# bcgsc/NanoSim

Measured on AMD Instinct MI355X. Metric: simulated reads/sec (genome mode, mean 8 kb), higher is better.
Workload: dtype u8

## Files before the change

### nanosim_amd/csrc/ns_chain.h

```cpp
#pragma once
#include "ns_device.h"

struct Tabs {
    const uint64_t *w;
    NS_DEV const double *d(uint32_t off) const { return reinterpret_cast<const double *>(w + off); }
    NS_DEV const uint64_t *q(uint32_t off) const { return w + off; }
    NS_DEV const uint16_t *h(uint32_t off) const { return reinterpret_cast<const uint16_t *>(w + off); }
    NS_DEV const uint32_t *u(uint32_t off) const { return reinterpret_cast<const uint32_t *>(w + off); }
    NS_DEV const int32_t *i(uint32_t off) const { return reinterpret_cast<const int32_t *>(w + off); }
};

template <class V>
NS_DEV int32_t ecdf_lookup_g(const double *__restrict__ hi, const V *__restrict__ vhi, uint32_t n,
                                                 double vlo0, const uint16_t *__restrict__ guide, uint32_t u) {
    double p = u32_to_p(u);
    uint32_t s = guide[u >> 24];
    if (s < n) {
        const double h0 = hi[s], h1 = hi[min(s + 1, n - 1)];
        if (p > h0) {
            ++s;
            if (s < n && p > h1) { ++s; while (s < n && p > hi[s]) ++s; }
        }
    }
    if (s >= n) { s = n - 1; p = hi[s]; }
    const uint32_t sm = s ? s - 1 : 0;
    const double hs = hi[s], hp = hi[sm], vs = (double)vhi[s], vp = (double)vhi[sm];
    const double plo = s ? hp : 0.0;
    const double vlo = s ? vp : vlo0;
    return (int32_t)floor((p - plo) / (hs - plo) * (vs - vlo) + vlo);
}

NS_DEV void mix_record(const Tabs &T, const ChainTab &c, uint32_t type, uint32_t comp, uint32_t &go, uint32_t &n, uint32_t &h) {
    const uint64_t *r = T.w + c.mix_rec + 2u * (2u * type + comp);
    const uint64_t r0 = r[0], r1 = r[1];
    go = (uint32_t)r0; n = (uint32_t)(r0 >> 32); h = (uint32_t)r1;
}
NS_DEV int32_t run_length_t(const Tabs &T, const ChainTab &c, int type, uint32_t u_mix, uint32_t u_len) {
    const int comp = ((uint64_t)u_mix < T.q(c.mix_w)[type]) ? 0 : 1;
    uint32_t go, n, h;
    mix_record(T, c, (uint32_t)type, (uint32_t)comp, go, n, h);
    const uint64_t u = u_len;
    uint32_t v = reinterpret_cast<const uint8_t *>(T.w)[8u * h + ns_clz32(~u_len)];
    while (v + 1 < n && u >= T.w[go + v]) ++v;
    return (int32_t)v + 1;
}

struct EvSink32 {
    ns_event *ev;
    uint32_t cap, n;
    int32_t shift;
    uint32_t last_ins_len;
    bool overflow;
    bool range;
    uint2 *stg;
    uint32_t stride;
};
#ifndef NS_CHAIN_BLOCK
#define NS_CHAIN_BLOCK 256
#endif
NS_DEV void ev_flush4(EvSink32 &s, uint32_t first) {
    const uint2 e0 = s.stg[0], e1 = s.stg[s.stride], e2 = s.stg[2u * s.stride], e3 = s.stg[3u * s.stride];
    uint4 *dst = reinterpret_cast<uint4 *>(s.ev + first);
    dst[0] = make_uint4(e0.x, e0.y, e1.x, e1.y); dst[1] = make_uint4(e2.x, e2.y, e3.x, e3.y);
}
NS_DEV void ev_flush_tail(EvSink32 &s) {
    if (s.stg && (s.n & 3u) && s.n < s.cap) ev_flush4(s, s.n & ~3u);
}
NS_DEV bool ev_shift_fits(int32_t shift) { return (uint32_t)(shift + NS_EV_SHIFT_BIAS) < 2u * (uint32_t)NS_EV_SHIFT_BIAS; }
NS_DEV void ev_push32(EvSink32 &s, int32_t pos, uint32_t type, int32_t len) {
    uint32_t l = len > (int32_t)NS_EV_LEN_MAX ? NS_EV_LEN_MAX : (uint32_t)len;
    if (len > (int32_t)NS_EV_LEN_MAX || !ev_shift_fits(s.shift)) s.range = true;
    if (s.n < s.cap) {
        ns_event e; e.pos = (uint32_t)pos; e.info = ns_ev_pack(l, type, s.shift);
        if (s.stg) {
            s.stg[(s.n & 3u) * s.stride] = make_uint2(e.pos, e.info);
            if ((s.n & 3u) == 3u) ev_flush4(s, s.n - 3u);
        } else s.ev[s.n] = e;
    } else s.overflow = true;
    if (type == NS_INS) { s.shift += (int32_t)l; s.last_ins_len = l; } else if (type == NS_DEL) s.shift -= (int32_t)l;
    s.n++;
}

struct EList32 { int32_t l_new, middle_ref; };

NS_DEV EList32 chain_error_list_g(const Tabs &T, const ChainTab &c, int32_t m_ref, const ns_key &key, uint32_t seg, uint32_t attempt, EvSink32 &s) {
    int32_t l_new = m_ref, pos = 0, middle_ref = m_ref;
    int state = NS_ST_START;
    u32x4 w = ns_draw(key, ST_EVENT, seg, attempt, 0, 0);
    int32_t prev_match = ecdf_lookup_g(T.d(c.fm_hi), T.d(c.fm_vhi), c.fm_n, c.fm_vlo0, T.h(c.fm_guide), w.x);
    if (prev_match < 2) prev_match = 2;
    pos += prev_match;
    uint32_t it = 1;
    int32_t last_ins_pos = -1;
    const uint64_t *trans = T.q(c.trans);
    const int32_t *bins = T.i(c.mm_bin);
    const uint32_t *seg_off = T.u(c.mm_seg_off);
    const uint8_t *bin_lut = reinterpret_cast<const uint8_t *>(T.w + c.mm_bin_lut);
    u32x4 w_next = ns_draw(key, ST_EVENT, seg, attempt, 1, 0);
    while (pos < middle_ref) {
        w = w_next;
        w_next = ns_draw(key, ST_EVENT, seg, attempt, it + 1, 0);
        const int error = trans_pick_u(trans + 3 * state, w.x);
        int32_t step = run_length_t(T, c, error, w.y, w.z);
        if (error == NS_INS) l_new += step; else if (error == NS_DEL) l_new -= step;
        if (error != NS_INS) {
            ev_push32(s, pos, (uint32_t)error, step);
            pos += step;
            if (pos >= middle_ref) { l_new += pos - middle_ref; middle_ref = pos; }
        } else {
            if (last_ins_pos == pos && s.n > 0) { s.n--; s.shift -= (int32_t)s.last_ins_len; }
            ev_push32(s, pos, NS_INS, step);
            last_ins_pos = pos;
        }
        state = NS_ST_MIS + error;
        uint32_t b;
        if ((uint32_t)prev_match < 256u) b = bin_lut[prev_match];
        else {
            for (b = 0; b < c.mm_nbins; ++b)
                if (bins[2 * b] <= prev_match && prev_match < bins[2 * b + 1]) break;
            if (b >= c.mm_nbins) b = c.mm_nbins - 1;
        }
        const uint32_t o = seg_off[b], ncol = seg_off[b + 1] - o;
        step = ecdf_lookup_g(T.d(c.mm_hi) + o, T.d(c.mm_vhi) + o, ncol, T.d(c.mm_vlo0)[b], T.h(c.mm_guide) + 256 * b, w.w);
        if (prev_match == 0 && step == 0) step = 1;
        prev_match = step;
        if (pos + prev_match > middle_ref) { l_new += pos + prev_match - middle_ref; middle_ref = pos + prev_match; }
        pos += prev_match;
        if (prev_match == 0) state += 3;
        else last_ins_pos = -1;
        ++it;
    }
    return EList32{l_new, middle_ref};
}

struct EvTrack { int32_t max_len, smin, smax; };
NS_DEV EvTrack ev_track_open(const EvSink32 &s) { return EvTrack{0, s.shift, s.shift}; }
NS_DEV void ev_track_close(EvSink32 &s, const EvTrack &t) {
    if (t.max_len > (int32_t)NS_EV_LEN_MAX || !ev_shift_fits(t.smin) || !ev_shift_fits(t.smax)) s.range = true;
    if (s.n > s.cap) s.overflow = true;
}
NS_DEV void ev_push32s(EvSink32 &s, EvTrack &t, int32_t pos, uint32_t type, int32_t len) {
    const uint32_t l = len > (int32_t)NS_EV_LEN_MAX ? NS_EV_LEN_MAX : (uint32_t)len;
    t.max_len = len > t.max_len ? len : t.max_len;
    t.smin = s.shift < t.smin ? s.shift : t.smin; t.smax = s.shift > t.smax ? s.shift : t.smax;
    if (s.n < s.cap) {
        ns_event e; e.pos = (uint32_t)pos; e.info = ns_ev_pack(l, type, s.shift);
        if (s.stg) {
            s.stg[(s.n & 3u) * s.stride] = make_uint2(e.pos, e.info);
            if ((s.n & 3u) == 3u) ev_flush4(s, s.n - 3u);
        } else s.ev[s.n] = e;
    }
    s.shift += type == NS_INS ? (int32_t)l : type == NS_DEL ? -(int32_t)l : 0;
    s.last_ins_len = type == NS_INS ? l : s.last_ins_len;
    s.n++;
}

NS_DEV int32_t run_length_r(const Tabs &T, const ChainTab &c, uint32_t type, uint64_t weight_thr, uint32_t u_mix, uint32_t u_len) {
    const uint32_t comp = (uint64_t)u_mix >= weight_thr ? 1u : 0u;
    const uint64_t *r = T.w + c.mix_rec + 2u * (2u * type + comp);
    const uint64_t r0 = r[0], r1 = r[1];
    const uint32_t go = (uint32_t)r0, rn = (uint32_t)(r0 >> 32);
    const uint64_t uz = u_len;
    uint32_t rv = reinterpret_cast<const uint8_t *>(T.w)[8u * (uint32_t)r1 + ns_clz32(~u_len)];
    const uint64_t ra = T.w[go + rv], rb = T.w[go + rv + 1u];
    const uint32_t c1 = (rv + 1u < rn ? 1u : 0u) & (uz >= ra ? 1u : 0u), c2 = c1 & (rv + 2u < rn ? 1u : 0u) & (uz >= rb ? 1u : 0u);
    rv += c1 + c2;
    if (c2) while (rv + 1u < rn && uz >= T.w[go + rv]) ++rv;
    return (int32_t)rv + 1;
}

#define NS_G_THR(g) ((g) & 0x1ffffffffull)
#define NS_GV_UNIT (1ull << 33)
#define NS_GV_NARROW (1ull << 34)
NS_DEV int32_t ecdf_lookup_gv(const uint64_t *__restrict__ GV, uint32_t n, const uint16_t *__restrict__ guide, uint32_t u,
                              const uint64_t *__restrict__ sub2, const double *__restrict__ hi_g, const double *__restrict__ vhi_g, double vlo0) {
    const uint32_t s0 = guide[u >> 24];
    const uint64_t uu = u;
    const uint32_t sc = min(s0, n - 1u);
    const uint64_t g0 = GV[sc], g1 = GV[sc + 1u];
    const uint32_t k0 = (s0 < n) & (uu >= NS_G_THR(g0)), k1 = k0 & (s0 + 1u < n) & (uu >= NS_G_THR(g1));
    uint64_t g = k0 ? g1 : g0;
    uint32_t s = s0 + k0 + k1;
    if (k1) {
        const uint32_t cell = u >> 24;
        uint32_t hi2 = cell < 255u ? min((uint32_t)guide[cell + 1u], n) : n;
        while (s < hi2) { const uint32_t mid = (s + hi2) >> 1; if (uu >= NS_G_THR(GV[mid])) s = mid + 1u; else hi2 = mid; }
        if (s < n) g = GV[s];
    }
    if (s < n && (g & NS_GV_UNIT)) return (int32_t)(uint32_t)(g >> 35) - 1;
    if (s < n && (g & NS_GV_NARROW)) {
        const uint64_t *t = sub2 + (g >> 35);
        const uint64_t h = t[0];
        const uint32_t nt = (uint32_t)(h >> 32);
        int32_t r = (int32_t)(uint32_t)h - (int32_t)nt;
        for (uint32_t k = 1; k <= nt; ++k) r += uu >= t[k] ? 1 : 0;
        return r;
    }
    double p = u32_to_p(u);
    if (s >= n) { s = n - 1; p = hi_g[s]; }
    const uint32_t sm = s ? s - 1 : 0;
    const double hs = hi_g[s], plo = s ? hi_g[sm] : 0.0, vs = vhi_g[s], vlo = s ? vhi_g[sm] : vlo0;
    return (int32_t)floor((p - plo) / (hs - plo) * (vs - vlo) + vlo);
}

NS_DEV bool ecdf_lookup_pre(const uint64_t *__restrict__ GV, uint32_t n, const uint16_t *__restrict__ guide, uint32_t u,
                            const uint64_t *__restrict__ sub2, int32_t &out) {
    const uint64_t uu = u;
    const uint32_t cell = u >> 24;
    uint32_t s = guide[cell], hi2 = cell < 255u ? min((uint32_t)guide[cell + 1u], n) : n;
    while (s < hi2) { const uint32_t mid = (s + hi2) >> 1; if (uu >= NS_G_THR(GV[mid])) s = mid + 1u; else hi2 = mid; }
    if (s >= n) return false;
    const uint64_t g = GV[s];
    if (g & NS_GV_UNIT) { out = (int32_t)(uint32_t)(g >> 35) - 1; return true; }
    if (g & NS_GV_NARROW) {
        const uint64_t *t = sub2 + (g >> 35);
        const uint64_t h = t[0];
        const uint32_t nt = (uint32_t)(h >> 32);
        int32_t r = (int32_t)(uint32_t)h - (int32_t)nt;
        for (uint32_t k = 1; k <= nt; ++k) r += uu >= t[k] ? 1 : 0;
        out = r;
        return true;
    }
    return false;
}
NS_DEV int32_t next_match_gv(const Tabs &T, const Tabs &TG, const ChainTab &c, int32_t prev_match, uint32_t u) {
    uint32_t b, o, ncol;
    if ((uint32_t)prev_match < 256u) {
        const uint64_t pp = T.q(c.pm_lut)[prev_match];
        int32_t r;
        if (ecdf_lookup_pre(T.q(c.mm_gv) + (uint32_t)pp, (uint32_t)(pp >> 32) & 0xffffffu, T.h(c.mm_guide) + 256u * (uint32_t)(pp >> 56), u, T.q(c.sub2), r)) return r;
        const uint64_t pe = TG.q(c.pm_full)[prev_match];
        b = (uint32_t)(pe >> 56); o = (uint32_t)pe; ncol = (uint32_t)(pe >> 32) & 0xffffffu;
    } else {
        const int32_t *bins = T.i(c.mm_bin);
        const uint32_t *seg_off = T.u(c.mm_seg_off);
        for (b = 0; b < c.mm_nbins; ++b)
            if (bins[2 * b] <= prev_match && prev_match < bins[2 * b + 1]) break;
        if (b >= c.mm_nbins) b = c.mm_nbins - 1;
        const uint64_t pp = T.q(c.pm_bin)[b];
        int32_t r;
        if (ecdf_lookup_pre(T.q(c.mm_gv) + (uint32_t)pp, (uint32_t)(pp >> 32) & 0xffffffu, T.h(c.mm_guide) + 256u * b, u, T.q(c.sub2), r)) return r;
        o = seg_off[b]; ncol = seg_off[b + 1] - o;
    }
    return ecdf_lookup_gv(TG.q(c.mm_gv_full) + o, ncol, T.h(c.mm_guide) + 256u * b, u, TG.q(c.sub2_full), TG.d(c.mm_hi) + o, TG.d(c.mm_vhi) + o, T.d(c.mm_vlo0)[b]);
}

NS_DEV EList32 chain_error_list(const Tabs &T, const Tabs &TG, const ChainTab &c, int32_t m_ref, const ns_key &key,
                                uint32_t seg, uint32_t attempt, EvSink32 &s) {
    int32_t l_new = m_ref, pos = 0, middle_ref = m_ref;
    uint32_t state = NS_ST_START;
    u32x4 w = ns_draw(key, ST_EVENT, seg, attempt, 0, 0);
    int32_t prev_match = ecdf_lookup_gv(TG.q(c.fm_gv), c.fm_n, T.h(c.fm_guide), w.x, TG.q(c.sub2_full), TG.d(c.fm_hi), TG.d(c.fm_vhi), c.fm_vlo0);
    if (prev_match < 2) prev_match = 2;
    pos += prev_match;
    uint32_t it = 1;
    int32_t last_ins_pos = -1;
    const uint64_t *trans = T.q(c.trans);
    const uint64_t *pm = T.q(c.pm_lut);
    const uint64_t *rec = T.q(c.mix_rec);
    const uint64_t *gv = T.q(c.mm_gv);
    const uint16_t *guide = T.h(c.mm_guide);
    const uint8_t *bytes = reinterpret_cast<const uint8_t *>(T.w);
    const uint64_t mw0 = T.q(c.mix_w)[0], mw1 = T.q(c.mix_w)[1], mw2 = T.q(c.mix_w)[2];
    u32x4 w_next = ns_draw(key, ST_EVENT, seg, attempt, 1, 0);
    EvTrack trk = ev_track_open(s);
    while (pos < middle_ref) {
        w = w_next;
        w_next = ns_draw(key, ST_EVENT, seg, attempt, it + 1, 0);
        const uint64_t ux = w.x, uy = w.y, uz = w.z, uw = w.w;
        const uint64_t t0 = trans[3u * state], t1 = trans[3u * state + 1u];
        const uint32_t small = (uint32_t)prev_match < 256u ? 1u : 0u;
        const uint64_t pe = pm[small ? (uint32_t)prev_match : 0u];
        const uint32_t e0 = ux >= t0 ? 1u : 0u, e1 = ux >= t1 ? 1u : 0u;
        const uint32_t error = e0 + (e0 & e1);
        const uint32_t b = (uint32_t)(pe >> 56), o = (uint32_t)pe, ncol = (uint32_t)(pe >> 32) & 0xffffffu;
        const uint64_t mw = error == NS_MIS ? mw0 : error == NS_INS ? mw1 : mw2;
        const uint32_t comp = uy >= mw ? 1u : 0u;
        const uint64_t r0 = rec[2u * (2u * error + comp)], r1 = rec[2u * (2u * error + comp) + 1u];
        const uint32_t s0 = guide[256u * b + (w.w >> 24)];
        const uint32_t go = (uint32_t)r0, rn = (uint32_t)(r0 >> 32);
        uint32_t rv = bytes[8u * (uint32_t)r1 + ns_clz32(~w.z)];
        const uint32_t sc = min(s0, ncol - 1u);
        const uint64_t g0 = gv[o + sc], g1 = gv[o + sc + 1u];
        const uint64_t ra = T.w[go + rv], rb = T.w[go + rv + 1u];
        const uint32_t k0 = (s0 < ncol ? 1u : 0u) & (uw >= NS_G_THR(g0) ? 1u : 0u), k1 = k0 & (s0 + 1u < ncol ? 1u : 0u) & (uw >= NS_G_THR(g1) ? 1u : 0u);
        const uint64_t g = k0 ? g1 : g0;
        const uint32_t fast = small & (s0 + k0 < ncol ? 1u : 0u) & (k1 ^ 1u) & ((g & NS_GV_UNIT) ? 1u : 0u);
        int32_t next = (int32_t)(uint32_t)(g >> 35) - 1;
        const uint32_t c1 = (rv + 1u < rn ? 1u : 0u) & (uz >= ra ? 1u : 0u), c2 = c1 & (rv + 2u < rn ? 1u : 0u) & (uz >= rb ? 1u : 0u);
        rv += c1 + c2;
        if (c2) while (rv + 1u < rn && uz >= T.w[go + rv]) ++rv;
        if (!fast) next = next_match_gv(T, TG, c, prev_match, w.w);
        const int32_t step = (int32_t)rv + 1;
        if (prev_match == 0 && next == 0) next = 1;
        const bool ins = error == NS_INS;
        l_new += ins ? step : error == NS_DEL ? -step : 0;
        const bool coll = ins && last_ins_pos == pos && s.n > 0;
        s.n -= coll ? 1u : 0u; s.shift -= coll ? (int32_t)s.last_ins_len : 0;
        ev_push32s(s, trk, pos, error, step);
        last_ins_pos = ins ? pos : last_ins_pos;
        pos += ins ? 0 : step;
        const bool over = !ins && pos >= middle_ref;
        l_new += over ? pos - middle_ref : 0; middle_ref = over ? pos : middle_ref;
        state = NS_ST_MIS + error;
        prev_match = next;
        if (pos + prev_match > middle_ref) { l_new += pos + prev_match - middle_ref; middle_ref = pos + prev_match; }
        pos += prev_match;
        if (prev_match == 0) state += 3;
        else last_ins_pos = -1;
        ++it;
    }
    ev_track_close(s, trk);
    return EList32{l_new, middle_ref};
}

NS_DEV EList32 chain_unaligned_error_list(const Tabs &T, const ChainTab &c, int32_t m_ref, const ns_key &key,
                                          uint32_t seg, uint32_t attempt, EvSink32 &s) {
    int32_t l_new = m_ref, pos = 0, middle_ref = m_ref;
    int32_t pend_ins = 0;
    if (m_ref <= 0) return EList32{l_new, middle_ref};
    uint32_t it = 0;
    u32x4 w_next = ns_draw(key, ST_UEVENT, seg, attempt, 0, 0);
    const uint64_t mw0 = T.q(c.mix_w)[0], mw1 = T.q(c.mix_w)[1], mw2 = T.q(c.mix_w)[2];
    EvTrack trk = ev_track_open(s);
    while (pos < middle_ref) {
        const u32x4 w = w_next;
        ++it;
        w_next = ns_draw(key, ST_UEVENT, seg, attempt, it, 0);
        const uint64_t ut = w.x;
        const uint32_t type = (ut < ns_thr_lt(0.4)) ? 3u : (ut < ns_thr_lt(0.7)) ? (uint32_t)NS_MIS : (ut < ns_thr_lt(0.85)) ? (uint32_t)NS_INS : (uint32_t)NS_DEL;
        const uint32_t tt = type == 3u ? (uint32_t)NS_MIS : type;
        const int32_t run = run_length_r(T, c, tt, tt == NS_MIS ? mw0 : tt == NS_INS ? mw1 : mw2, w.y, w.z);
        const int32_t step = type == 3u ? 1 : run;
        const bool is_ins = type == NS_INS, is_mis = type == NS_MIS, is_del = type == NS_DEL;
        l_new += is_ins ? step : is_del ? -step : 0;
        const int32_t L = is_ins ? 0 : pend_ins;
        pend_ins = is_ins ? pend_ins + step : 0;
        const bool va = is_mis || is_del;
        int32_t dl = step - L; dl = dl < 1 ? 1 : dl;
        const int32_t la = L == 0 ? step : is_mis ? 1 : dl;
        const int32_t lb = is_del ? L - (step - 1) : L;
        const bool vb = L > 0 && lb > 0;
        const bool vc = is_mis && L > 0 && step - 1 > L;
        if (va) ev_push32s(s, trk, pos, type, la);
        if (vb) ev_push32s(s, trk, pos + 1, NS_INS, lb);
        if (vc) ev_push32s(s, trk, pos + 1, NS_MIS, step - 1 - L);
        pos += is_ins ? 0 : step;
        const bool over = pos > middle_ref;
        l_new += over ? pos - middle_ref : 0; middle_ref = over ? pos : middle_ref;
    }
    ev_track_close(s, trk);
    return EList32{l_new, middle_ref};
}

__device__ inline EList32 coop_unaligned_error_list(const Tabs &T, const ChainTab &c, int32_t m_ref, const ns_key &key, uint32_t seg,
                                                    uint32_t attempt, EvSink32 &s, uint32_t lane) {
    int32_t l_new = m_ref, middle_ref = m_ref;
    if (m_ref <= 0) return EList32{l_new, middle_ref};
    uint32_t pos0 = 0, pend0 = 0;
    auto draw = [&](uint32_t it, int &type, uint32_t &step) {
        const u32x4 w = ns_draw(key, ST_UEVENT, seg, attempt, it, 0);
        const uint64_t ut = w.x;
        type = (ut < ns_thr_lt(0.4)) ? 3 : (ut < ns_thr_lt(0.7)) ? NS_MIS : (ut < ns_thr_lt(0.85)) ? NS_INS : NS_DEL;
        step = 1;
        if (type != 3) step = (uint32_t)run_length_t(T, c, type, w.y, w.z);
    };
    int type_n; uint32_t step_n;
    draw(lane, type_n, step_n);
    for (uint32_t it0 = 0;; it0 += 64) {
        int type = type_n; uint32_t step = step_n;
        draw(it0 + 64 + lane, type_n, step_n);
        const uint32_t adv = type == NS_INS ? 0u : step;
        const uint32_t adv_incl = wave_incl_scan(adv);
        const uint32_t pos = pos0 + adv_incl - adv;
        const bool exec = pos < (uint32_t)m_ref;
// ... 156 lines not shown
        s.n += n_blk;
        l_new += (int32_t)ins_tot - (int32_t)del_tot;
        uint32_t pend1 = pend0 + ins_tot;
        if (HAS) {
            const int jl = 63 - __clzll((long long)HAS);
            pend1 = (uint32_t)__shfl((int)run, jl) + ins_tot - (uint32_t)__shfl((int)i_incl, jl);
        }
        s.shift = (int32_t)((uint32_t)s.shift + (pend0 + ins_tot - pend1) - del_tot);
        pend0 = pend1;
        pos0 += adv_tot;
        if (n_ran < 64u * K || pos0 >= (uint32_t)m_ref) break;
    }
    if (__ballot(bad)) s.range = true;
    if ((int32_t)pos0 > middle_ref) { l_new += (int32_t)pos0 - middle_ref; middle_ref = (int32_t)pos0; }
    return EList32{l_new, middle_ref};
}

#define COOP_MAX_BINS 16u
struct CoopLds {
    uint32_t err_tab[64];
    uint16_t step_tab[64][4];
    uint32_t match_tab[64][COOP_MAX_BINS];
    ns_event ev_buf[64];
};

__device__ inline EList32 coop_error_list(const Tabs &TM, const Tabs &T, const ChainTab &c, int32_t m_ref, const ns_key &key, uint32_t seg,
                                          uint32_t attempt, EvSink32 &s, CoopLds &S, uint32_t lane) {
    int32_t l_new = m_ref, pos = 0, middle_ref = m_ref;
    int state = NS_ST_START;
    u32x4 w = ns_draw(key, ST_EVENT, seg, attempt, 0, 0);
    int32_t prev_match = ecdf_lookup_g(T.d(c.fm_hi), T.d(c.fm_vhi), c.fm_n, c.fm_vlo0, T.h(c.fm_guide), w.x);
    if (prev_match < 2) prev_match = 2;
    pos += prev_match;
    uint32_t it0 = 1;
    int32_t last_ins_pos = -1;
    const uint64_t *trans = TM.q(c.trans);
    const int32_t *bins = T.i(c.mm_bin);
    const uint32_t *seg_off = T.u(c.mm_seg_off);
    const uint8_t *bin_lut = reinterpret_cast<const uint8_t *>(T.w + c.mm_bin_lut);
    auto bin_of = [&](int32_t v) -> uint32_t {
        if ((uint32_t)v < 256u) return bin_lut[v];
        uint32_t b = 0;
        for (; b < c.mm_nbins; ++b)
            if (bins[2 * b] <= v && v < bins[2 * b + 1]) break;
        return b >= c.mm_nbins ? c.mm_nbins - 1 : b;
    };
    uint32_t pbin = bin_of(prev_match);
    while (pos < middle_ref) {
        {
            const u32x4 wi = ns_draw(key, ST_EVENT, seg, attempt, it0 + lane, 0);
            uint32_t eb = 0;
#pragma unroll
            for (int st = 0; st < 7; ++st) eb |= (uint32_t)trans_pick_u(trans + 3 * st, wi.x) << (2 * st);
            S.err_tab[lane] = eb;
#pragma unroll
            for (int t = 0; t < 3; ++t) S.step_tab[lane][t] = (uint16_t)run_length_t(TM, c, t, wi.y, wi.z);
            if (c.int_image) {
                const uint16_t *g16 = T.h(c.mm_g16);
                const uint64_t *gvf = T.q(c.mm_gv_full);
                const uint32_t cell = wi.w >> 16, nb = c.mm_nbins;
                const uint64_t uu = wi.w;
                for (uint32_t b0 = 0; b0 < nb; b0 += 4) {
                    uint32_t o[4], nc[4], s0[4];
                    uint64_t ga[4], gb[4];
#pragma unroll
                    for (uint32_t k = 0; k < 4; ++k) {
                        const uint32_t b = min(b0 + k, nb - 1u);
                        o[k] = seg_off[b]; nc[k] = seg_off[b + 1] - o[k];
                        s0[k] = g16[(size_t)b * 65536u + cell];
                    }
#pragma unroll
                    for (uint32_t k = 0; k < 4; ++k) {
                        const uint32_t sc = min(s0[k], nc[k] ? nc[k] - 1u : 0u);
                        ga[k] = gvf[o[k] + sc]; gb[k] = gvf[o[k] + sc + 1u];
                    }
#pragma unroll
                    for (uint32_t k = 0; k < 4; ++k) {
                        const uint32_t b = min(b0 + k, nb - 1u);
                        const uint32_t k0 = (s0[k] < nc[k] ? 1u : 0u) & (uu >= NS_G_THR(ga[k]) ? 1u : 0u);
                        const uint32_t k1 = k0 & (s0[k] + 1u < nc[k] ? 1u : 0u) & (uu >= NS_G_THR(gb[k]) ? 1u : 0u);
                        const uint64_t g = k0 ? gb[k] : ga[k];
                        int32_t v = (int32_t)(uint32_t)(g >> 35) - 1;
                        if (!((s0[k] + k0 < nc[k]) && !k1 && (g & NS_GV_UNIT)))
                            v = ecdf_lookup_gv(gvf + o[k], nc[k], T.h(c.mm_guide) + 256u * b, wi.w, T.q(c.sub2_full), T.d(c.mm_hi) + o[k], T.d(c.mm_vhi) + o[k], T.d(c.mm_vlo0)[b]);
                        if (b0 + k < nb) S.match_tab[lane][b0 + k] = (uint32_t)(uint16_t)v | bin_of(v) << 16 | bin_of(v == 0 ? 1 : v) << 24;
                    }
                }
            } else
            for (uint32_t b = 0; b < c.mm_nbins; ++b) {
                const uint32_t o = seg_off[b];
                const int32_t v = ecdf_lookup_g(T.d(c.mm_hi) + o, T.d(c.mm_vhi) + o, seg_off[b + 1] - o, T.d(c.mm_vlo0)[b], T.h(c.mm_guide) + 256 * b, wi.w);
                S.match_tab[lane][b] = (uint32_t)(uint16_t)v | bin_of(v) << 16 | bin_of(v == 0 ? 1 : v) << 24;
            }
        }
        __builtin_amdgcn_fence(__ATOMIC_ACQ_REL, "wavefront");
        __builtin_amdgcn_wave_barrier();
        uint32_t nl = 0;
        uint32_t i = 0;
        for (; i < 64 && pos < middle_ref; ++i) {
            const int error = (int)((S.err_tab[i] >> (2 * state)) & 3u);
            int32_t step = S.step_tab[i][error];
            if (error == NS_INS) l_new += step; else if (error == NS_DEL) l_new -= step;
            int32_t epos = pos;
            if (error != NS_INS) {
                pos += step;
                if (pos >= middle_ref) { l_new += pos - middle_ref; middle_ref = pos; }
            } else {
                if (last_ins_pos == pos && (nl > 0 || s.n > 0)) {
                    if (nl > 0) --nl; else --s.n;
                    s.shift -= (int32_t)s.last_ins_len;
                }
                last_ins_pos = pos;
            }
            {
                const uint32_t l = step > (int32_t)NS_EV_LEN_MAX ? NS_EV_LEN_MAX : (uint32_t)step;
                if (step > (int32_t)NS_EV_LEN_MAX || !ev_shift_fits(s.shift)) s.range = true;
                ns_event e; e.pos = (uint32_t)epos; e.info = ns_ev_pack(l, (uint32_t)error, s.shift);
                if (lane == 0) S.ev_buf[nl] = e;
                ++nl;
                if (error == NS_INS) { s.shift += (int32_t)l; s.last_ins_len = l; } else if (error == NS_DEL) s.shift -= (int32_t)l;
            }
            state = NS_ST_MIS + error;
            const uint32_t me = S.match_tab[i][pbin];
            step = (int32_t)(me & 0xffffu);
            pbin = (me >> 16) & 0xffu;
            if (prev_match == 0 && step == 0) { step = 1; pbin = me >> 24; }
            prev_match = step;
            if (pos + prev_match > middle_ref) { l_new += pos + prev_match - middle_ref; middle_ref = pos + prev_match; }
            pos += prev_match;
            if (prev_match == 0) state += 3;
            else last_ins_pos = -1;
        }
        __builtin_amdgcn_fence(__ATOMIC_ACQ_REL, "wavefront");
        __builtin_amdgcn_wave_barrier();
        if (lane < nl) {
            if (s.n + lane < s.cap) s.ev[s.n + lane] = S.ev_buf[lane];
        }
        if (s.n + nl > s.cap) s.overflow = true;
        s.n += nl;
        it0 += i;
        __builtin_amdgcn_fence(__ATOMIC_ACQ_REL, "wavefront");
        __builtin_amdgcn_wave_barrier();
    }
    return EList32{l_new, middle_ref};
}
```

### nanosim_amd/csrc/ns_device.h

```cpp
#pragma once
#include "ns_rng.h"
#include "../../include/nanosim_amd.h"

enum NsStat : uint32_t {
    NS_STAT_OVER,
    NS_STAT_BASES,
    NS_STAT_REF_BASES,
    NS_STAT_EVENTS,
    NS_STAT_MAX_READ,
    NS_STAT_HP_FAILED,
    NS_STAT_NEXT_N,
    NS_STAT_HP_OVER,
    NS_STAT_COUNT
};
#define NS_RANGE_SHIFT 40
#define NS_OVER_MASK ((1ull << NS_RANGE_SHIFT) - 1)
#define NS_STATS_WAYS 64u
#define NS_STATS_BYTES ((NS_STAT_COUNT + NS_STAT_COUNT * NS_STATS_WAYS) * sizeof(unsigned long long))
__host__ __device__ inline unsigned long long *ns_stats_way(unsigned long long *stats, uint32_t way) { return stats + NS_STAT_COUNT + NS_STAT_COUNT * way; }

struct ChainTab {
    uint32_t n_words;
    uint32_t trans;
    uint32_t mix_w;
// ... 16 lines not shown
struct DevModel {
    uint32_t flags;
    ChainTab ct;
    const uint64_t *chain_blob;
    uint32_t fm_nseg;
    const double *fm_hi, *fm_vhi;
    double fm_vlo0;
    uint32_t mm_nbins;
    const int64_t *mm_bin_lo, *mm_bin_hi;
    const uint32_t *mm_seg_off;
    const double *mm_hi, *mm_vhi, *mm_vlo0;
    double trans[7][3];
    double mix_w[3];
    uint32_t mix_n[3][2];
    const double *mix_cdf[3][2];
    ns_kde kde[NS_KDE_COUNT];
    double strandness_rate;
    uint32_t nseg_n;
    const double *nseg_cdf;
    const uint32_t *qual_thr;
    const uint16_t *qual_lut;
    ns_hp_class hp[2];
    double hp_mis_rate;
    const double *kde2d_x, *kde2d_y;
    uint64_t kde2d_n;
    double kde2d_bw;
};

struct DevTrx {
    uint32_t n_expr;
    const uint32_t *expr_chrom;
    const double *expr_cum;
    const uint8_t *polya;
    double polya_scale;
};

struct DevRef {
    const uint8_t *bases;
    const uint64_t *chrom_off;
    const uint8_t *circular;
    const char *names;
    const uint32_t *name_off;
    uint32_t nchrom;
    const uint8_t *spliced;
};

NS_DEV int64_t ecdf_lookup(const double *__restrict__ hi, const double *__restrict__ vhi,
                           uint32_t n, double vlo0, double p) {
    uint32_t lo_i = 0, hi_i = n;
    while (lo_i < hi_i) {
        uint32_t mid = (lo_i + hi_i) >> 1;
        if (p <= hi[mid]) hi_i = mid; else lo_i = mid + 1;
    }
    uint32_t s = lo_i;
    if (s >= n) { s = n - 1; p = hi[s]; }
    double plo = s ? hi[s - 1] : 0.0;
    double vlo = s ? vhi[s - 1] : vlo0;
    return (int64_t)floor((p - plo) / (hi[s] - plo) * (vhi[s] - vlo) + vlo);
}

NS_DEV int64_t table_value(const double *__restrict__ cdf, uint32_t n, double p) {
    uint32_t lo = 0, hi = n;
    while (lo < hi) {
        uint32_t mid = (lo + hi) >> 1;
        if (p <= cdf[mid]) hi = mid; else lo = mid + 1;
    }
    if (lo >= n) lo = n - 1;
    return (int64_t)lo + 1;
}

__host__ __device__ inline uint64_t ns_thr_lt(double t) {
    if (!(t > 0.0)) return 0;
    if (t >= 1.0) return 1ull << 32;
    const double y = ceil(t * 4294967296.0 - 0.5);
    return y <= 0.0 ? 0ull : (uint64_t)y;
}
__host__ __device__ inline uint64_t ns_thr_gt(double t) {
    if (t < 0.0) return 0;
    if (t >= 1.0) return 1ull << 32;
    const double y = floor(t * 4294967296.0 - 0.5) + 1.0;
    return y <= 0.0 ? 0ull : (uint64_t)y;
}

NS_DEV int trans_pick_u(const uint64_t *row, uint32_t u) {
    return (uint64_t)u < row[0] ? NS_MIS : (uint64_t)u < row[1] ? NS_INS : NS_DEL;
}

__device__ __forceinline__ double kde_sample(const ns_kde &k, const u32x4 &w) {
    uint64_t i = (uint64_t)(u53_to_p(w.x, w.y) * (double)k.n);
    if (i >= k.n) i = k.n - 1;
    return fma(k.bw, ns_norminv(u32_to_p(w.z)), k.data[i]);
}

__device__ inline bool seg_length(const DevModel &m, const ns_params &prm, const ns_key &key, uint32_t s,
                                  uint32_t epoch, int64_t &out) {
    for (uint32_t j = 0; j < NS_KDE_RETRY; ++j) {
        u32x4 w = ns_draw(key, ST_REFLEN, s, epoch, j, 0);
        double x;
        if (!prm.use_lognormal) x = kde_sample(m.kde[NS_KDE_ALIGNED], w);
        else if (prm.kind == NS_KIND_PERFECT)
            x = ns_exp(fma(prm.sd_len, ns_norminv(u32_to_p(w.z)), ns_log(prm.median_len)));
        else {
            u32x4 w2 = ns_draw(key, ST_REFLEN, s, epoch, j, 1);
            double tot = ns_exp(fma(prm.sd_len, ns_norminv(u32_to_p(w.z)),
                                    ns_log(prm.median_len + prm.sd_len * prm.sd_len / 2)));
            double rem = ns_pow10m1(kde_sample(m.kde[NS_KDE_HT], w2));
            if (rem < 0) continue;
            x = tot - rem;
        }
        bool keep = (prm.kind == NS_KIND_PERFECT) ? ((double)prm.min_len <= x && x <= (double)prm.max_len)
                                                  : (0 < x && x <= (double)prm.max_len);
        if (keep) { out = (int64_t)x; return true; }
    }
    return false;
}
__device__ inline int64_t gap_length(const DevModel &m, const ns_key &key, uint32_t g, uint32_t epoch) {
    u32x4 w = ns_draw(key, ST_GAPLEN, g, epoch, 0, 0);
    int64_t gi = ns_f64_to_i64_sat(ns_pow10m1(kde_sample(m.kde[NS_KDE_GAP], w)));
    return gi < 0 ? 0 : gi;
}
__device__ inline int64_t unaligned_length(const DevModel &m, const ns_params &prm, const ns_key &key, uint32_t a) {
    u32x4 w = ns_draw(key, ST_ULEN, 0, a, 0, 0);
    double x = prm.use_lognormal ? ns_exp(fma(prm.sd_len, ns_norminv(u32_to_p(w.z)), ns_log(prm.median_len)))
                                 : kde_sample(m.kde[NS_KDE_UNALIGNED], w);
    const int64_t v = ns_len_draw(x);
    return v > prm.max_len ? -1 : v;
}

__device__ inline bool extract_pos(const DevRef &ref, int64_t length, const ns_key &key, uint32_t seg, uint32_t attempt,
                                   uint32_t &chrom, uint64_t &pos) {
    uint64_t genome_len = ref.chrom_off[ref.nchrom];
    for (uint32_t j = 0; j < NS_POS_RETRY; ++j) {
        u32x4 w = ns_draw(key, ST_POS, seg, attempt, j, 0);
        uint64_t ref_pos = (uint64_t)(u53_to_p(w.x, w.y) * (double)(genome_len + 1));
        if (ref_pos > genome_len) ref_pos = genome_len;
        if (ref.circular[0]) { chrom = 0; pos = ref_pos; return true; }
        if (length > 0 && ref.nchrom > 8) {
            uint32_t lo = 0, hi = ref.nchrom;
            while (hi - lo > 1) { const uint32_t mid = (lo + hi) >> 1; if (ref.chrom_off[mid] <= ref_pos) lo = mid; else hi = mid; }
            const uint64_t local = ref_pos - ref.chrom_off[lo], cl = ref.chrom_off[lo + 1] - ref.chrom_off[lo];
            if (local + (uint64_t)length <= cl) { chrom = lo; pos = local; return true; }
            continue;
        }
        for (uint32_t c = 0; c < ref.nchrom; ++c) {
            uint64_t cl = ref.chrom_off[c + 1] - ref.chrom_off[c];
            if (ref_pos + (uint64_t)length <= cl) { chrom = c; pos = ref_pos; return true; }
            else if (ref_pos < cl) break;
            else ref_pos -= cl;
        }
    }
    return false;
}

__device__ inline uint32_t trx_pick(const DevTrx &tx, double u) {
    const double v = u * tx.expr_cum[tx.n_expr - 1];
    uint32_t lo = 0, hi = tx.n_expr - 1;
    while (lo < hi) { const uint32_t mid = (lo + hi) >> 1; if (v < tx.expr_cum[mid]) hi = mid; else lo = mid + 1; }
    return lo;
}
__device__ inline int64_t kde2d_cond(const DevModel &m, double L, const ns_key &key, uint32_t attempt, uint32_t sub) {
    const double *__restrict__ x = m.kde2d_x, *__restrict__ y = m.kde2d_y;
    const double h = m.kde2d_bw;
    const uint64_t n = m.kde2d_n;
    uint64_t lo, hi;
    { uint64_t a = 0, b = n; const double v = L - 5.0 * h; while (a < b) { const uint64_t md = (a + b) >> 1; if (x[md] < v) a = md + 1; else b = md; } lo = a; }
    { uint64_t a = lo, b = n; const double v = L + 5.0 * h; while (a < b) { const uint64_t md = (a + b) >> 1; if (x[md] <= v) a = md + 1; else b = md; } hi = a; }
// ... 181 lines not shown
```

### nanosim_amd/csrc/ns_pack.h

```cpp
#pragma once
#include <math.h>
#define NS_PACK_THR(g) ((g) & 0x1ffffffffull)
#include <string.h>
#include <vector>
#include "ns_device.h"

static inline void ns_pack_chain_tables(const ns_model_tables *t, uint32_t nseg, ChainTab &ct, std::vector<uint64_t> &blob, bool &whole,
                                        uint32_t force_tail_bits = 0) {
    blob.clear();
    auto put_d = [&](const double *src, size_t n) { uint32_t off = (uint32_t)blob.size(); blob.resize(off + n);
                                                     memcpy(blob.data() + off, src, n * 8); return off; };
    auto put_raw = [&](const void *src, size_t bytes) { uint32_t off = (uint32_t)blob.size(); blob.resize(off + (bytes + 7) / 8, 0);
                                                         memcpy(blob.data() + off, src, bytes); return off; };
    auto put_q = [&](const std::vector<uint64_t> &v) { uint32_t off = (uint32_t)blob.size(); blob.insert(blob.end(), v.begin(), v.end()); return off; };
    auto guide = [&](const double *hi, uint32_t n) {
        std::vector<uint16_t> g(256);
        uint32_t sidx = 0;
        for (uint32_t i = 0; i < 256; ++i) {
            double edge = (double)i / 256.0;
            while (sidx < n && hi[sidx] < edge) ++sidx;
            g[i] = (uint16_t)(sidx > 65535u ? 65535u : sidx);
        }
        return g;
    };
    auto put_thr = [&](const double *src, size_t n, bool gt) {
        uint32_t off = (uint32_t)blob.size(); blob.resize(off + n);
        for (size_t i = 0; i < n; ++i) blob[off + i] = gt ? ns_thr_gt(src[i]) : ns_thr_lt(src[i]);
        return off; };
    whole = true;
    ct.trans = put_thr(&t->trans[0][0], 21, false);
    ct.mix_w = put_thr(t->mix_w, 3, false);
    uint64_t rec[12];
    for (int ty = 0; ty < 3; ++ty)
        for (int c = 0; c < 2; ++c) {
            const uint32_t nn = t->mix_n[ty][c];
            const uint32_t cdf = put_thr(t->mix_cdf[ty][c], nn, true);
            uint8_t g2[40] = {0};
            const uint64_t *G = blob.data() + cdf;
            for (uint32_t l = 0; l <= 32; ++l) {
                const uint64_t lo_u = l == 0 ? 0ull : (0xffffffffull << (32 - l)) & 0xffffffffull;
                uint32_t v = 0;
                while (v + 1 < nn && lo_u >= G[v]) ++v;
                g2[l] = (uint8_t)(v > 255u ? 255u : v);
            }
            const uint32_t gd = put_raw(g2, 40);
            rec[2 * (2 * ty + c)] = (uint64_t)cdf | (uint64_t)nn << 32;
            rec[2 * (2 * ty + c) + 1] = gd;
        }
    ct.mix_rec = put_raw(rec, sizeof rec);
    ct.n_words_mix = (uint32_t)blob.size();
    ct.fm_n = t->fm_nseg; ct.fm_vlo0 = t->fm_vlo0;
    { auto g = guide(t->fm_hi, t->fm_nseg); ct.fm_guide = put_raw(g.data(), 512); }
    ct.mm_nbins = t->mm_nbins;
    std::vector<int32_t> bins(2 * (size_t)t->mm_nbins);
    for (uint32_t b = 0; b < t->mm_nbins; ++b) {
        auto clamp = [](int64_t v) { return (int32_t)(v > 0x7fffffff ? 0x7fffffff : v < -0x7fffffff ? -0x7fffffff : v); };
        bins[2 * b] = clamp(t->mm_bin_lo[b]); bins[2 * b + 1] = clamp(t->mm_bin_hi[b]);
    }
    ct.mm_bin = put_raw(bins.data(), bins.size() * 4);
    std::vector<uint8_t> lut(256);
    for (int v = 0; v < 256; ++v) {
        uint32_t b = 0;
        for (; b < t->mm_nbins; ++b) if (bins[2 * b] <= v && v < bins[2 * b + 1]) break;
        if (b >= t->mm_nbins) b = t->mm_nbins - 1;
        lut[v] = (uint8_t)b;
    }
    ct.mm_bin_lut = put_raw(lut.data(), 256);
    ct.mm_seg_off = put_raw(t->mm_seg_off, ((size_t)t->mm_nbins + 1) * 4);
    ct.mm_vlo0 = put_d(t->mm_vlo0, t->mm_nbins);
    std::vector<uint16_t> gall;
    for (uint32_t b = 0; b < t->mm_nbins; ++b) {
        auto g = guide(t->mm_hi + t->mm_seg_off[b], t->mm_seg_off[b + 1] - t->mm_seg_off[b]);
        gall.insert(gall.end(), g.begin(), g.end());
    }
    ct.mm_guide = put_raw(gall.data(), gall.size() * 2);
    auto segments = [&](const double *hi, const double *src, size_t n, double vlo0, std::vector<uint64_t> &out, std::vector<uint64_t> &sub2) {
        for (size_t i = 0; i < n; ++i) {
            if (!(src[i] >= 0 && src[i] < 536870912.0 && src[i] == floor(src[i]))) whole = false;
            const uint32_t e = (uint32_t)(src[i] < 0 ? 0 : src[i] >= 2147483647.0 ? 2147483647.0 : src[i]);
            const double hs = hi[i], plo = i ? hi[i - 1] : 0.0, vs = src[i], vlo = i ? src[i - 1] : vlo0;
            const double w = vs - vlo;
            uint64_t word = ns_thr_gt(hs);
            if (w >= 1.0 && w <= 15.0 && w == floor(w) && hs > plo && vlo == floor(vlo) && vlo >= 0) {
                auto f = [&](uint64_t u) { const double pp = u32_to_p((uint32_t)u); return floor((pp - plo) / (hs - plo) * (vs - vlo) + vlo); };
                const uint64_t u0 = i ? ns_thr_gt(plo) : 0ull, u1 = ns_thr_gt(hs);
                uint64_t thr[15];
                for (uint32_t k = 1; k <= (uint32_t)w; ++k) {
                    uint64_t lo = u0, hi2 = u1;
                    while (lo < hi2) { const uint64_t mid = lo + ((hi2 - lo) >> 1); if (f(mid) >= vlo + (double)k) hi2 = mid; else lo = mid + 1; }
                    thr[k - 1] = lo >= u1 ? (1ull << 32) : lo;
                }
                if (w == 1.0 && thr[0] == (1ull << 32)) word |= 1ull << 33 | (uint64_t)e << 35;
                else {
                    word |= 1ull << 34 | (uint64_t)sub2.size() << 35;
                    sub2.push_back((uint64_t)e | (uint64_t)(uint32_t)w << 32);
                    sub2.insert(sub2.end(), thr, thr + (uint32_t)w);
                }
            }
            out.push_back(word);
        } };
    std::vector<uint64_t> fm_gv, mm_full, sub2_full;
    segments(t->fm_hi, t->fm_vhi, t->fm_nseg, t->fm_vlo0, fm_gv, sub2_full);
    for (uint32_t b = 0; b < t->mm_nbins; ++b) {
        const uint32_t o = t->mm_seg_off[b];
        segments(t->mm_hi + o, t->mm_vhi + o, t->mm_seg_off[b + 1] - o, t->mm_vlo0[b], mm_full, sub2_full);
    }
    if (sub2_full.size() >= (1u << 28)) whole = false;
    sub2_full.push_back(0);
    std::vector<uint64_t> pm_full(256);
    for (uint32_t v = 0; v < 256; ++v) {
        const uint32_t b = lut[v], o = t->mm_seg_off[b], nc = t->mm_seg_off[b + 1] - o;
        if (nc >= (1u << 24)) whole = false;
        pm_full[v] = (uint64_t)o | (uint64_t)(nc & 0xffffffu) << 32 | (uint64_t)b << 56;
    }
    const size_t head_words = blob.size();
    auto prefix_len = [&](uint32_t b, uint32_t bits) {
        const uint32_t o = t->mm_seg_off[b], nc = t->mm_seg_off[b + 1] - o;
        if (!bits) return nc;
        const uint64_t cut = (1ull << 32) - (1ull << (32 - bits));
        uint32_t r = 0;
        while (r < nc && NS_PACK_THR(mm_full[o + r]) < cut) ++r;
        return r < nc ? r + 1 : nc;
    };
    auto image_words = [&](uint32_t tb) {
        size_t n = head_words + 256 + 64 + t->mm_nbins + sub2_full.size();
        for (uint32_t b = 0; b < t->mm_nbins; ++b) n += prefix_len(b, tb);
        return n; };
    uint32_t bits = 0;
    if (image_words(0) * 8 > 24 * 1024) {
        bits = 8;
        for (uint32_t limit : {24u * 1024u, 44u * 1024u}) {
            uint32_t best = 0;
            for (uint32_t tb = 14; tb >= (limit == 24u * 1024u ? 12u : 8u); --tb) if (image_words(tb) * 8 <= limit) { best = tb; break; }
            if (best) { bits = best; break; }
        }
// ... 59 lines not shown
```

Measured before the change: 122.0 million.

## Use octave-based log-spaced ECDF guide cells and inline narrow-table lookup

Replaces the uniform 256-cell guide table for ECDF lookups with a log-spaced layout (32 cells per octave of leading ones, 8 octaves). This gives finer resolution near p→1, where CDF thresholds cluster, so the guide lands closer and fewer binary-search steps are needed. The chain loop also handles the NARROW sub-table case inline instead of calling the full next_match_gv fallback. It adds optional counter hooks, but they compile away by default. The guide tables keep the same total size (256 cells), but each cell index now costs a clz and extra shifts to compute.

```diff
diff --git a/nanosim_amd/csrc/ns_chain.h b/nanosim_amd/csrc/ns_chain.h
--- a/nanosim_amd/csrc/ns_chain.h
+++ b/nanosim_amd/csrc/ns_chain.h
@@ -14,7 +14,7 @@
 NS_DEV int32_t ecdf_lookup_g(const double *__restrict__ hi, const V *__restrict__ vhi, uint32_t n,
                                                  double vlo0, const uint16_t *__restrict__ guide, uint32_t u) {
     double p = u32_to_p(u);
-    uint32_t s = guide[u >> 24];
+    uint32_t s = guide[guide_cell(u)];
     if (s < n) {
         const double h0 = hi[s], h1 = hi[min(s + 1, n - 1)];
         if (p > h0) {
@@ -121,7 +121,7 @@
             if (b >= c.mm_nbins) b = c.mm_nbins - 1;
         }
         const uint32_t o = seg_off[b], ncol = seg_off[b + 1] - o;
-        step = ecdf_lookup_g(T.d(c.mm_hi) + o, T.d(c.mm_vhi) + o, ncol, T.d(c.mm_vlo0)[b], T.h(c.mm_guide) + 256 * b, w.w);
+        step = ecdf_lookup_g(T.d(c.mm_hi) + o, T.d(c.mm_vhi) + o, ncol, T.d(c.mm_vlo0)[b], T.h(c.mm_guide) + NS_GUIDE_CELLS * b, w.w);
         if (prev_match == 0 && step == 0) step = 1;
         prev_match = step;
         if (pos + prev_match > middle_ref) { l_new += pos + prev_match - middle_ref; middle_ref = pos + prev_match; }
@@ -170,11 +170,15 @@
 }
 
 #define NS_G_THR(g) ((g) & 0x1ffffffffull)
+#ifndef NS_CHAIN_COUNT
+#define NS_CHAIN_COUNT(what)
+#endif
+enum { NS_CNT_ITER, NS_CNT_FALLBACK, NS_CNT_NARROW, NS_CNT_K1, NS_CNT_N };
 #define NS_GV_UNIT (1ull << 33)
 #define NS_GV_NARROW (1ull << 34)
 NS_DEV int32_t ecdf_lookup_gv(const uint64_t *__restrict__ GV, uint32_t n, const uint16_t *__restrict__ guide, uint32_t u,
                               const uint64_t *__restrict__ sub2, const double *__restrict__ hi_g, const double *__restrict__ vhi_g, double vlo0) {
-    const uint32_t s0 = guide[u >> 24];
+    const uint32_t cell = guide_cell(u), s0 = guide[cell];
     const uint64_t uu = u;
     const uint32_t sc = min(s0, n - 1u);
     const uint64_t g0 = GV[sc], g1 = GV[sc + 1u];
@@ -182,8 +186,7 @@
     uint64_t g = k0 ? g1 : g0;
     uint32_t s = s0 + k0 + k1;
     if (k1) {
-        const uint32_t cell = u >> 24;
-        uint32_t hi2 = cell < 255u ? min((uint32_t)guide[cell + 1u], n) : n;
+        uint32_t hi2 = cell + 1u < NS_GUIDE_CELLS ? min((uint32_t)guide[cell + 1u], n) : n;
         while (s < hi2) { const uint32_t mid = (s + hi2) >> 1; if (uu >= NS_G_THR(GV[mid])) s = mid + 1u; else hi2 = mid; }
         if (s < n) g = GV[s];
     }
@@ -206,8 +209,8 @@
 NS_DEV bool ecdf_lookup_pre(const uint64_t *__restrict__ GV, uint32_t n, const uint16_t *__restrict__ guide, uint32_t u,
                             const uint64_t *__restrict__ sub2, int32_t &out) {
     const uint64_t uu = u;
-    const uint32_t cell = u >> 24;
-    uint32_t s = guide[cell], hi2 = cell < 255u ? min((uint32_t)guide[cell + 1u], n) : n;
+    const uint32_t cell = guide_cell(u);
+    uint32_t s = guide[cell], hi2 = cell + 1u < NS_GUIDE_CELLS ? min((uint32_t)guide[cell + 1u], n) : n;
     while (s < hi2) { const uint32_t mid = (s + hi2) >> 1; if (uu >= NS_G_THR(GV[mid])) s = mid + 1u; else hi2 = mid; }
     if (s >= n) return false;
     const uint64_t g = GV[s];
@@ -228,7 +231,7 @@
     if ((uint32_t)prev_match < 256u) {
         const uint64_t pp = T.q(c.pm_lut)[prev_match];
         int32_t r;
-        if (ecdf_lookup_pre(T.q(c.mm_gv) + (uint32_t)pp, (uint32_t)(pp >> 32) & 0xffffffu, T.h(c.mm_guide) + 256u * (uint32_t)(pp >> 56), u, T.q(c.sub2), r)) return r;
+        if (ecdf_lookup_pre(T.q(c.mm_gv) + (uint32_t)pp, (uint32_t)(pp >> 32) & 0xffffffu, T.h(c.mm_guide) + NS_GUIDE_CELLS * (uint32_t)(pp >> 56), u, T.q(c.sub2), r)) return r;
         const uint64_t pe = TG.q(c.pm_full)[prev_match];
         b = (uint32_t)(pe >> 56); o = (uint32_t)pe; ncol = (uint32_t)(pe >> 32) & 0xffffffu;
     } else {
@@ -239,10 +242,10 @@
         if (b >= c.mm_nbins) b = c.mm_nbins - 1;
         const uint64_t pp = T.q(c.pm_bin)[b];
         int32_t r;
-        if (ecdf_lookup_pre(T.q(c.mm_gv) + (uint32_t)pp, (uint32_t)(pp >> 32) & 0xffffffu, T.h(c.mm_guide) + 256u * b, u, T.q(c.sub2), r)) return r;
+        if (ecdf_lookup_pre(T.q(c.mm_gv) + (uint32_t)pp, (uint32_t)(pp >> 32) & 0xffffffu, T.h(c.mm_guide) + NS_GUIDE_CELLS * b, u, T.q(c.sub2), r)) return r;
         o = seg_off[b]; ncol = seg_off[b + 1] - o;
     }
-    return ecdf_lookup_gv(TG.q(c.mm_gv_full) + o, ncol, T.h(c.mm_guide) + 256u * b, u, TG.q(c.sub2_full), TG.d(c.mm_hi) + o, TG.d(c.mm_vhi) + o, T.d(c.mm_vlo0)[b]);
+    return ecdf_lookup_gv(TG.q(c.mm_gv_full) + o, ncol, T.h(c.mm_guide) + NS_GUIDE_CELLS * b, u, TG.q(c.sub2_full), TG.d(c.mm_hi) + o, TG.d(c.mm_vhi) + o, T.d(c.mm_vlo0)[b]);
 }
 
 NS_DEV EList32 chain_error_list(const Tabs &T, const Tabs &TG, const ChainTab &c, int32_t m_ref, const ns_key &key,
@@ -277,7 +280,7 @@
         const uint64_t mw = error == NS_MIS ? mw0 : error == NS_INS ? mw1 : mw2;
         const uint32_t comp = uy >= mw ? 1u : 0u;
         const uint64_t r0 = rec[2u * (2u * error + comp)], r1 = rec[2u * (2u * error + comp) + 1u];
-        const uint32_t s0 = guide[256u * b + (w.w >> 24)];
+        const uint32_t s0 = guide[NS_GUIDE_CELLS * b + guide_cell(w.w)];
         const uint32_t go = (uint32_t)r0, rn = (uint32_t)(r0 >> 32);
         uint32_t rv = bytes[8u * (uint32_t)r1 + ns_clz32(~w.z)];
         const uint32_t sc = min(s0, ncol - 1u);
@@ -285,12 +288,27 @@
         const uint64_t ra = T.w[go + rv], rb = T.w[go + rv + 1u];
         const uint32_t k0 = (s0 < ncol ? 1u : 0u) & (uw >= NS_G_THR(g0) ? 1u : 0u), k1 = k0 & (s0 + 1u < ncol ? 1u : 0u) & (uw >= NS_G_THR(g1) ? 1u : 0u);
         const uint64_t g = k0 ? g1 : g0;
-        const uint32_t fast = small & (s0 + k0 < ncol ? 1u : 0u) & (k1 ^ 1u) & ((g & NS_GV_UNIT) ? 1u : 0u);
+        const uint32_t found = small & (s0 + k0 < ncol ? 1u : 0u) & (k1 ^ 1u);
+        const uint32_t fast = found & ((g & NS_GV_UNIT) ? 1u : 0u);
         int32_t next = (int32_t)(uint32_t)(g >> 35) - 1;
         const uint32_t c1 = (rv + 1u < rn ? 1u : 0u) & (uz >= ra ? 1u : 0u), c2 = c1 & (rv + 2u < rn ? 1u : 0u) & (uz >= rb ? 1u : 0u);
         rv += c1 + c2;
         if (c2) while (rv + 1u < rn && uz >= T.w[go + rv]) ++rv;
-        if (!fast) next = next_match_gv(T, TG, c, prev_match, w.w);
+        NS_CHAIN_COUNT(NS_CNT_ITER);
+        if (k1) NS_CHAIN_COUNT(NS_CNT_K1);
+        if (!fast) {
+            if (found && (g & NS_GV_NARROW)) {
+                const uint64_t *t = T.q(c.sub2) + (g >> 35);
+                const uint64_t h = t[0];
+                const uint32_t nt = (uint32_t)(h >> 32);
+                next = (int32_t)(uint32_t)h - (int32_t)nt;
+                for (uint32_t k = 1; k <= nt; ++k) next += uw >= t[k] ? 1 : 0;
+                NS_CHAIN_COUNT(NS_CNT_NARROW);
+            } else {
+                next = next_match_gv(T, TG, c, prev_match, w.w);
+                NS_CHAIN_COUNT(NS_CNT_FALLBACK);
+            }
+        }
         const int32_t step = (int32_t)rv + 1;
         if (prev_match == 0 && next == 0) next = 1;
         const bool ins = error == NS_INS;
@@ -613,14 +631,14 @@
                         const uint64_t g = k0 ? gb[k] : ga[k];
                         int32_t v = (int32_t)(uint32_t)(g >> 35) - 1;
                         if (!((s0[k] + k0 < nc[k]) && !k1 && (g & NS_GV_UNIT)))
-                            v = ecdf_lookup_gv(gvf + o[k], nc[k], T.h(c.mm_guide) + 256u * b, wi.w, T.q(c.sub2_full), T.d(c.mm_hi) + o[k], T.d(c.mm_vhi) + o[k], T.d(c.mm_vlo0)[b]);
+                            v = ecdf_lookup_gv(gvf + o[k], nc[k], T.h(c.mm_guide) + NS_GUIDE_CELLS * b, wi.w, T.q(c.sub2_full), T.d(c.mm_hi) + o[k], T.d(c.mm_vhi) + o[k], T.d(c.mm_vlo0)[b]);
                         if (b0 + k < nb) S.match_tab[lane][b0 + k] = (uint32_t)(uint16_t)v | bin_of(v) << 16 | bin_of(v == 0 ? 1 : v) << 24;
                     }
                 }
             } else
             for (uint32_t b = 0; b < c.mm_nbins; ++b) {
                 const uint32_t o = seg_off[b];
-                const int32_t v = ecdf_lookup_g(T.d(c.mm_hi) + o, T.d(c.mm_vhi) + o, seg_off[b + 1] - o, T.d(c.mm_vlo0)[b], T.h(c.mm_guide) + 256 * b, wi.w);
+                const int32_t v = ecdf_lookup_g(T.d(c.mm_hi) + o, T.d(c.mm_vhi) + o, seg_off[b + 1] - o, T.d(c.mm_vlo0)[b], T.h(c.mm_guide) + NS_GUIDE_CELLS * b, wi.w);
                 S.match_tab[lane][b] = (uint32_t)(uint16_t)v | bin_of(v) << 16 | bin_of(v == 0 ? 1 : v) << 24;
             }
         }
diff --git a/nanosim_amd/csrc/ns_device.h b/nanosim_amd/csrc/ns_device.h
--- a/nanosim_amd/csrc/ns_device.h
+++ b/nanosim_amd/csrc/ns_device.h
@@ -122,6 +122,20 @@
     return y <= 0.0 ? 0ull : (uint64_t)y;
 }
 
+#ifndef NS_GUIDE_OCTAVES
+#define NS_GUIDE_OCTAVES 8u
+#endif
+#define NS_GUIDE_CELLS (32u * NS_GUIDE_OCTAVES)
+NS_HD uint32_t guide_cell(uint32_t u) {
+    const uint32_t ones = ns_clz32(~u);
+    const uint32_t last = ones >= NS_GUIDE_OCTAVES - 1u ? 1u : 0u, l = last ? NS_GUIDE_OCTAVES - 1u : ones;
+    return 32u * l + ((u >> (26u + last - l)) & 31u);
+}
+NS_HD uint32_t guide_cell_start(uint32_t cell) {
+    const uint32_t l = cell >> 5, m = cell & 31u, last = l == NS_GUIDE_OCTAVES - 1u ? 1u : 0u;
+    return (uint32_t)(0xffffffff00000000ull >> l) | m << (26u + last - l);
+}
+
 NS_DEV int trans_pick_u(const uint64_t *row, uint32_t u) {
     return (uint64_t)u < row[0] ? NS_MIS : (uint64_t)u < row[1] ? NS_INS : NS_DEL;
 }
diff --git a/nanosim_amd/csrc/ns_pack.h b/nanosim_amd/csrc/ns_pack.h
--- a/nanosim_amd/csrc/ns_pack.h
+++ b/nanosim_amd/csrc/ns_pack.h
@@ -14,10 +14,10 @@
                                                          memcpy(blob.data() + off, src, bytes); return off; };
     auto put_q = [&](const std::vector<uint64_t> &v) { uint32_t off = (uint32_t)blob.size(); blob.insert(blob.end(), v.begin(), v.end()); return off; };
     auto guide = [&](const double *hi, uint32_t n) {
-        std::vector<uint16_t> g(256);
+        std::vector<uint16_t> g(NS_GUIDE_CELLS);
         uint32_t sidx = 0;
-        for (uint32_t i = 0; i < 256; ++i) {
-            double edge = (double)i / 256.0;
+        for (uint32_t i = 0; i < NS_GUIDE_CELLS; ++i) {
+            double edge = (double)guide_cell_start(i) * 0x1p-32;
             while (sidx < n && hi[sidx] < edge) ++sidx;
             g[i] = (uint16_t)(sidx > 65535u ? 65535u : sidx);
         }
@@ -50,7 +50,7 @@
     ct.mix_rec = put_raw(rec, sizeof rec);
     ct.n_words_mix = (uint32_t)blob.size();
     ct.fm_n = t->fm_nseg; ct.fm_vlo0 = t->fm_vlo0;
-    { auto g = guide(t->fm_hi, t->fm_nseg); ct.fm_guide = put_raw(g.data(), 512); }
+    { auto g = guide(t->fm_hi, t->fm_nseg); ct.fm_guide = put_raw(g.data(), g.size() * 2); }
     ct.mm_nbins = t->mm_nbins;
     std::vector<int32_t> bins(2 * (size_t)t->mm_nbins);
     for (uint32_t b = 0; b < t->mm_nbins; ++b) {
```

New measurement: 125.6 million (median of 6 runs). 3.0% higher.
